# GANtastic3/MaskCycleGAN-VC

Measured on AMD Instinct MI355X. Metric: train iters/s (full G+D step), 80x64 mel bs=1, higher is better.
Workload: dtype f32

## Files before the change

### maskcyclegan-vc_amd/csrc/trunk.h

```cpp
#pragma once
#include <hip/hip_runtime.h>

enum TrunkMode { TRUNK_PLAIN = 0, TRUNK_IN = 1, TRUNK_IN_GLU = 2 };

struct TrunkArgs {
    const float* a0; const float* a1;
    const float* bias0; const float* bias1;
    const float* x; long long x_sc; long long x_sb;
    int Cin, KW, K;
    int M, Mtot;
    int B, T4, N;
    float* conv_out; long long c_sc; long long c_sb;
    int accumulate;
    int slab_all;
    float* slabs; long long slab_stride;
    float* stats;
    const float* gamma0; const float* beta0; const float* gamma1; const float* beta1;
    float* y; const float* res; long long y_sn; long long y_sc;
    float eps;
    int mode;
    int pre;
    int pre_C;
    const float* pre_x;
    int pre_xB;
// ... 17 lines not shown
    float* stats;
    float* y; long long y_sn, y_sc;
    const float* res;
    int Cin, KW, M, mode;
    int rows;
};
#define MCVC_TRUNK_NET_LAYERS 13
struct TrunkFwdNetArgs {
    TrunkLayerDesc L[MCVC_TRUNK_NET_LAYERS];
    int nlayers, B, T4;
    int x_floats;
    float eps;
    unsigned* sync;
    int fault_inject;
};
int mcvc_trunk_set_fault_inject(int on);
int mcvc_trunk_set_passes_in_flight(int n);
bool mcvc_trunk_net_applies(int B, int T4);
int mcvc_trunk_fwd_net_launch(TrunkFwdNetArgs& a, hipStream_t s);
#define MCVC_TRUNK_SYNC_WORDS 32

struct TrunkBwdLayerDesc {
    const float* wt;
    const float* dy;
    const float* px;
    int pxB;
    const float* stats;
    const float* g0; const float* b0; const float* g1; const float* b1;
    float* xout;
    float* dg0; float* db0; float* dg1; float* db1;
    float* out;
    int pre, C, M, rows;
    int flags;
};
enum { TBWD_ACCUMULATE = 1,
       TBWD_DY_FRESH = 2,
       TBWD_SLAB_DY = 4, TBWD_SLAB_OUT = 8 };
#define MCVC_TRUNK_BWD_LAYERS 12
struct TrunkBwdNetArgs {
    TrunkBwdLayerDesc L[MCVC_TRUNK_BWD_LAYERS];
    int nlayers, B, T4, x_floats;
    const float* slabs; long long slab_stride; int nslab;
    unsigned* sync;
    unsigned* err;
    int fault_inject;
};
bool mcvc_trunk_bwd_net_applies(int B, int T4);
int mcvc_trunk_bwd_net_launch(TrunkBwdNetArgs& a, hipStream_t s);
```

### maskcyclegan-vc_amd/csrc/trunk_kernels.hip

```cpp
#include "mcvc_common.h"
#include "trace.h"
#include "launch.h"
#include "trunk.h"

#define MFMA16(a, b, c) __builtin_amdgcn_mfma_f32_16x16x4f32((a), (b), (c), 0, 0, 0)

namespace {

constexpr int kTrunkWaves = 8;
constexpr int kTrunkThreads = 64 * kTrunkWaves;

__host__ __device__ inline int trunk_doff(int KW) { return KW == 3 ? 4 : 0; }
__host__ __device__ inline int trunk_tp(int T4, int KW) { return T4 + trunk_doff(KW); }
__host__ __device__ inline int trunk_rs(int B, int T4, int KW)
{
    int rs = B * trunk_tp(T4, KW);
    if (KW == 3) { while ((rs & 7) != 4) ++rs; }
    else { while ((rs & 3) != 2) ++rs; }
    return rs;
}
__host__ __device__ inline int trunk_na(int N) { return (N + 15) >> 4; }
constexpr int kRedPitch = 80;
__host__ __device__ inline int trunk_epi_floats(int NA) { return kTrunkWaves * NA * 4 * kRedPitch + 16 * (16 * NA + 1) + 16 * 8 * 2 + 16; }

// ... 600 lines not shown
                if (!ok) __hip_atomic_store(a.sync + MCVC_TRUNK_SYNC_WORDS - 1, 1u + (unsigned)l, __ATOMIC_RELAXED, __HIP_MEMORY_SCOPE_AGENT);
                flag[0] = ok ? 1.f : 0.f;
            }
            asm volatile("s_waitcnt lgkmcnt(0)" ::: "memory");
            __builtin_amdgcn_s_barrier();
            if (flag[0] == 0.f) {
                const TrunkLayerDesc& dl = a.L[a.nlayers - 1];
                const int N = a.B * a.T4;
                for (int tile = blockIdx.x; tile < dl.M / dl.rows; tile += gridDim.x)
                    for (int i = tid; i < dl.rows * N; i += kNetThreads) {
                        const int row = i / N, col = i - row * N, b = col / a.T4, t = col - b * a.T4;
                        dl.y[(long long)b * dl.y_sn + (long long)(tile * dl.rows + row) * dl.y_sc + t] = __builtin_nanf("");
                    }
                return;
            }
        }
        if (d.KW == 3) net_stage_x<3>(d.x, Xs, d.Cin, a.B, a.T4, tid, l > 0); else net_stage_x<1>(d.x, Xs, d.Cin, a.B, a.T4, tid, l > 0);
        __syncthreads();
        const bool wt = (l + 1 < a.nlayers);
        for (int tile = blockIdx.x; tile < ntiles; tile += gridDim.x) {
            if (tile != (int)blockIdx.x) { if (d.KW == 3) net_load_w<3>(d, tile, w3); else net_load_w<1>(d, tile, w1); net_load_e(d, a.B, a.T4, tile, pe); }
            if (d.KW == 3) net_tile<3, NA>(d, a.B, a.T4, a.eps, tile, Xs, epi, wt, w3, pe);
            else net_tile<1, NA>(d, a.B, a.T4, a.eps, tile, Xs, epi, wt, w1, pe);
        }
        if (wt) {
            asm volatile("s_waitcnt vmcnt(0)" ::: "memory");
            __syncthreads();
            if (tid == 0 && !(a.fault_inject && l == 0 && blockIdx.x == 0))
                __hip_atomic_fetch_add(a.sync + l, 1u, __ATOMIC_RELAXED, __HIP_MEMORY_SCOPE_AGENT);
        }
    }
}

__device__ __forceinline__ void bnet_stage_pre(const TrunkBwdNetArgs& a, const TrunkBwdLayerDesc& d, float* Xs, float* rsum, int B, int T4, int tid)
{
    constexpr int DOFF = 4;
    const int TP = T4 + DOFF, RS = trunk_rs(B, T4, 3);
    const int C = d.C;
    const bool pglu = (d.pre == 2);
    const int Cx = pglu ? 2 * C : C;
    const int PB = d.pxB > 0 ? d.pxB : B;
    const float invT = 1.0f / (float)T4;
    const int E = (T4 + 3) >> 2;
    const int items = Cx * B * 4;
    const int nwg = (int)gridDim.x, me = (int)blockIdx.x;
    if (T4 == 16 && !(d.flags & TBWD_SLAB_DY) && ((reinterpret_cast<unsigned long long>(d.dy) | reinterpret_cast<unsigned long long>(d.px) |
                                                   reinterpret_cast<unsigned long long>(d.xout)) & 15ull) == 0) {
        constexpr int U = 4;
        const bool fresh = (d.flags & TBWD_DY_FRESH) != 0;
        const __amdgpu_buffer_rsrc_t rs = __builtin_amdgcn_make_buffer_rsrc(const_cast<float*>(d.dy), 0, C * B * 16 * 4, 0x00020000);
        for (int it0 = 0; it0 < items; it0 += U * kNetThreads) {
            float4 vd[U], v0[U], v1[U];
            float g0[U], b0[U], g1[U], b1[U], m0[U], r0[U], m1[U], r1[U];
#pragma unroll
            for (int u = 0; u < U; ++u) {
                const int item = it0 + u * kNetThreads + tid;
                const bool live = item < items;
                const int q4 = item & 3, row = live ? (item >> 2) : 0;
                const int cx = row / B, b = row - cx * B;
                const bool gate = pglu && cx >= C;
                const int c = gate ? cx - C : cx;
                const long long ro = ((long long)c * B + b) * 16 + q4 * 4;
                const long long po = ((long long)c * PB + b) * 16 + q4 * 4;
                vd[u] = fresh ? __builtin_bit_cast(float4, __builtin_amdgcn_raw_buffer_load_b128(rs, (int)(ro * 4), 0, 16))
                              : *reinterpret_cast<const float4*>(d.dy + ro);
                v0[u] = *reinterpret_cast<const float4*>(d.px + po);
                v1[u] = pglu ? *reinterpret_cast<const float4*>(d.px + po + (long long)C * PB * 16) : make_float4(0.f, 0.f, 0.f, 0.f);
                g0[u] = d.g0[c]; b0[u] = d.b0[c];
                g1[u] = pglu ? d.g1[c] : 0.f; b1[u] = pglu ? d.b1[c] : 0.f;
                const float* st = d.stats + (long long)b * Cx * 2;
                m0[u] = st[2 * c]; r0[u] = st[2 * c + 1];
                m1[u] = pglu ? st[2 * (c + C)] : 0.f; r1[u] = pglu ? st[2 * (c + C) + 1] : 1.f;
            }
#pragma unroll
            for (int u = 0; u < U; ++u) {
                const int item = it0 + u * kNetThreads + tid;
                const bool live = item < items;
                const int q4 = item & 3, row = live ? (item >> 2) : 0;
                const int cx = row / B, b = row - cx * B;
                const bool gate = pglu && cx >= C;
                const float dv[4] = {vd[u].x, vd[u].y, vd[u].z, vd[u].w};
                const float x0[4] = {v0[u].x, v0[u].y, v0[u].z, v0[u].w};
                const float x1[4] = {v1[u].x, v1[u].y, v1[u].z, v1[u].w};
                float dzv[4], xhv[4];
                float s1 = 0.f, s2 = 0.f;
#pragma unroll
                for (int e = 0; e < 4; ++e) {
                    const float xh0 = (x0[e] - m0[u]) * r0[u];
                    float dz, xh;
                    if (pglu) {
                        const float xh1 = (x1[e] - m1[u]) * r1[u];
                        const float sg = sigmoidf_(xh1 * g1[u] + b1[u]);
                        if (gate) { dz = dv[e] * (xh0 * g0[u] + b0[u]) * sg * (1.0f - sg); xh = xh1; }
                        else { dz = dv[e] * sg; xh = xh0; }
                    } else { dz = dv[e]; xh = xh0; }
                    dzv[e] = live ? dz : 0.f; xhv[e] = live ? xh : 0.f;
                    s1 += dzv[e]; s2 += dzv[e] * xhv[e];
                }
                s1 += __shfl_xor(s1, 1, 64); s2 += __shfl_xor(s2, 1, 64);
                s1 += __shfl_xor(s1, 2, 64); s2 += __shfl_xor(s2, 2, 64);
                if (live) {
                    const bool mine = (cx % nwg) == me;
                    const float gr = gate ? g1[u] * r1[u] : g0[u] * r0[u];
                    float o[4];
#pragma unroll
                    for (int e = 0; e < 4; ++e) o[e] = gr * (dzv[e] - s1 * invT - xhv[e] * (s2 * invT));
                    *reinterpret_cast<float4*>(Xs + cx * RS + b * TP + DOFF + q4 * 4) = make_float4(o[0], o[1], o[2], o[3]);
                    if (mine) *reinterpret_cast<float4*>(d.xout + ((long long)cx * B + b) * 16 + q4 * 4) = make_float4(o[0], o[1], o[2], o[3]);
                    if (q4 == 0 && mine) { rsum[((cx / nwg) * B + b) * 2] = s1; rsum[((cx / nwg) * B + b) * 2 + 1] = s2; }
                }
            }
        }
    } else
    for (int it0 = 0; it0 < items; it0 += kNetThreads) {
        const int item = it0 + tid;
        const bool live = item < items;
        const int q4 = item & 3, row = live ? (item >> 2) : 0;
        const int cx = row / B, b = row - cx * B;
        const bool gate = pglu && cx >= C;
        const int c = gate ? cx - C : cx;
        const float g0 = d.g0[c], b0 = d.b0[c];
        const float g1 = pglu ? d.g1[c] : 0.f, b1 = pglu ? d.b1[c] : 0.f;
        const float* st = d.stats + (long long)b * Cx * 2;
        const float m0 = st[2 * c], r0 = st[2 * c + 1];
        const float m1 = pglu ? st[2 * (c + C)] : 0.f, r1 = pglu ? st[2 * (c + C) + 1] : 1.f;
        const int t0 = q4 * E;
        const float* dyr = d.dy + ((long long)c * B + b) * T4 + t0;
        const float* x0r = d.px + ((long long)c * PB + b) * T4 + t0;
        const float* x1r = d.px + ((long long)(c + C) * PB + b) * T4 + t0;
        float vd[8], v0[8], v1[8];
#pragma unroll
        for (int e = 0; e < 8; ++e) {
            const bool ok = live && e < E && (t0 + e) < T4;
            vd[e] = ok ? ((d.flags & TBWD_DY_FRESH) ? __hip_atomic_load(dyr + e, __ATOMIC_RELAXED, __HIP_MEMORY_SCOPE_AGENT) : dyr[e]) : 0.f;
            if (ok && (d.flags & TBWD_SLAB_DY))
                for (int sl = 1; sl < a.nslab; ++sl) vd[e] += a.slabs[(long long)(sl - 1) * a.slab_stride + ((long long)c * B + b) * T4 + t0 + e];
            v0[e] = ok ? x0r[e] : 0.f; v1[e] = (ok && pglu) ? x1r[e] : 0.f;
        }
        float dzv[8], xhv[8];
        float s1 = 0.f, s2 = 0.f;
#pragma unroll
        for (int e = 0; e < 8; ++e) {
            const bool ok = e < E && (t0 + e) < T4;
            const float xh0 = (v0[e] - m0) * r0;
            float dz, xh;
            if (pglu) {
                const float xh1 = (v1[e] - m1) * r1;
                const float sg = sigmoidf_(xh1 * g1 + b1);
                if (gate) { dz = vd[e] * (xh0 * g0 + b0) * sg * (1.0f - sg); xh = xh1; }
                else { dz = vd[e] * sg; xh = xh0; }
            } else { dz = vd[e]; xh = xh0; }
            dzv[e] = ok ? dz : 0.f; xhv[e] = ok ? xh : 0.f;
            s1 += dzv[e]; s2 += dzv[e] * xhv[e];
        }
        s1 += __shfl_xor(s1, 1, 64); s2 += __shfl_xor(s2, 1, 64);
        s1 += __shfl_xor(s1, 2, 64); s2 += __shfl_xor(s2, 2, 64);
        if (live) {
            const bool mine = (cx % nwg) == me;
            const float gr = gate ? g1 * r1 : g0 * r0;
            float* xrow = Xs + cx * RS + b * TP + DOFF;
            float* od = mine ? (d.xout + ((long long)cx * B + b) * T4 + t0) : nullptr;
#pragma unroll
            for (int e = 0; e < 8; ++e) {
                if (e < E && (t0 + e) < T4) {
                    const float dxv = gr * (dzv[e] - s1 * invT - xhv[e] * (s2 * invT));
                    xrow[t0 + e] = dxv;
                    if (od) od[e] = dxv;
                }
            }
            if (q4 == 0 && mine) { rsum[((cx / nwg) * B + b) * 2] = s1; rsum[((cx / nwg) * B + b) * 2 + 1] = s2; }
        }
    }
    trunk_zero_gaps(Xs, Cx, B, TP, RS, DOFF, tid, kNetThreads);
    __syncthreads();
    for (int j = tid; j * nwg + me < Cx; j += kNetThreads) {
        const int cx = j * nwg + me;
        const bool gate = pglu && cx >= C;
        const int c = gate ? cx - C : cx;
        float dgam = 0.f, dbet = 0.f;
        for (int b = 0; b < B; ++b) { dbet += rsum[(j * B + b) * 2]; dgam += rsum[(j * B + b) * 2 + 1]; }
        float* dg = gate ? d.dg1 : d.dg0;
        float* db = gate ? d.db1 : d.db0;
        if (dg) dg[c] += dgam;
        if (db) db[c] += dbet;
    }
}

template <int NA>
__device__ __forceinline__ void bnet_tile(const TrunkBwdLayerDesc& d, int B, int T4, int tile, const float* Xs, float* epi, bool wt,
                                          NetW<3>& pre, float old)
{
    constexpr int KW = 3, DOFF = 4;
    const int tid = threadIdx.x;
    const int lane = tid & 63;
    const int wave = __builtin_amdgcn_readfirstlane(tid >> 6);
    const int l15 = lane & 15, kq = lane >> 4;
    const int TP = T4 + DOFF, RS = trunk_rs(B, T4, 3);
    const int N = B * T4;
    const int Cx = (d.pre == 2) ? 2 * d.C : d.C;
    const int K = Cx * KW;
    const int rows = d.rows, r0 = tile * rows;
    const int k_count = K / kNetWaves;
    const int k_begin = wave * k_count;
    const float* arow = d.wt + (long long)(r0 + (l15 < rows ? l15 : rows - 1)) * K;
    constexpr int NQ = 3, GK = 48, CH = 4;
    const int sgroups = k_count / GK;
    const float* ap = arow + k_begin + 4 * NQ * kq;
    float4 (&wb)[CH][3] = pre.wb;
    int off[NA][NQ][4];
#pragma unroll
    for (int h = 0; h < NA; ++h) {
        const int n = l15 + 16 * h;
        int xcol = B * TP, live = 0;
        if (n < N) { const int b = n / T4, t = n - b * T4; xcol = b * TP + DOFF - 1 + t; live = 1; }
#pragma unroll
        for (int q = 0; q < NQ; ++q)
#pragma unroll
            for (int j = 0; j < 4; ++j) {
                const int kr = 4 * (NQ * kq + q) + j;
                off[h][q][j] = (kr / KW) * RS + xcol + (live ? (kr % KW) : 0);
            }
    }
    f32x4 acc[NA];
#pragma unroll
    for (int h = 0; h < NA; ++h) acc[h] = f32x4{0.f, 0.f, 0.f, 0.f};
    {
        const float* xs = Xs + (k_begin / KW) * RS;
        for (int sg0 = 0; sg0 < sgroups; sg0 += CH) {
            if (sg0 > 0) {
#pragma unroll
                for (int c = 0; c < CH; ++c) {
                    const float* pp = ap + (long long)(sg0 + c < sgroups ? sg0 + c : 0) * GK;
#pragma unroll
                    for (int q = 0; q < NQ; ++q) wb[c][q] = *reinterpret_cast<const float4*>(pp + 4 * q);
                }
            }
#pragma unroll
            for (int c = 0; c < CH; ++c) {
                if (sg0 + c < sgroups) {
                    float xv[NQ][4][NA];
#pragma unroll
                    for (int q = 0; q < NQ; ++q)
#pragma unroll
                        for (int j = 0; j < 4; ++j)
#pragma unroll
                            for (int h = 0; h < NA; ++h) xv[q][j][h] = xs[off[h][q][j]];
#pragma unroll
                    for (int q = 0; q < NQ; ++q) {
                        const float av[4] = {wb[c][q].x, wb[c][q].y, wb[c][q].z, wb[c][q].w};
#pragma unroll
                        for (int j = 0; j < 4; ++j)
#pragma unroll
                            for (int h = 0; h < NA; ++h) acc[h] = MFMA16(av[j], xv[q][j][h], acc[h]);
                    }
                    __builtin_amdgcn_sched_group_barrier(0x100, NQ * 4 * NA, 0);
                    __builtin_amdgcn_sched_group_barrier(0x008, NQ * 4 * NA, 0);
                    xs += (GK / KW) * RS;
                }
            }
        }
    }
    float* red = epi;
#pragma unroll
    for (int h = 0; h < NA; ++h)
#pragma unroll
        for (int r = 0; r < 4; ++r) red[((wave * NA + h) * 4 + r) * kRedPitch + lane] = acc[h][r];
    __syncthreads();
    if (tid < rows * N) {
        const int mrow = tid / N, col = tid - mrow * N;
        const int h = col >> 4, ln = ((mrow >> 2) << 4) + (col & 15), r = mrow & 3;
        float v = 0.f;
#pragma unroll
        for (int w = 0; w < kNetWaves; ++w) v += red[((w * NA + h) * 4 + r) * kRedPitch + ln];
        if (d.flags & TBWD_ACCUMULATE) v += old;
        float* dst = d.out + (long long)(r0 + mrow) * N + col;
        if (wt) st_wt(dst, v); else *dst = v;
    }
}

static_assert(sizeof(Twin<TrunkBwdNetArgs>) <= 4096 && sizeof(Twin<TrunkFwdNetArgs>) <= 4096, "kernel arguments are limited to 4 KB");
template <int NA>
__global__ void __launch_bounds__(kNetThreads) trunk_bwd_net_kernel(const Twin<TrunkBwdNetArgs> tw)
{
    const TrunkBwdNetArgs& a = tw.v[blockIdx.z];
    extern __shared__ __attribute__((aligned(16))) float smem[];
    float* Xs = smem;
    float* rsum = smem + a.x_floats;
    float* epi = rsum + 16 * 8 * 2 * 2;
    float* flag = epi + kNetWaves * NA * 4 * kRedPitch;
    const int tid = threadIdx.x;
    const int N = a.B * a.T4;
    for (int l = 0; l < a.nlayers; ++l) {
        const TrunkBwdLayerDesc d = a.L[l];
        const int ntiles = d.M / d.rows;
        const int Cx = (d.pre == 2) ? 2 * d.C : d.C;
        NetW<3> w3;
        TrunkLayerDesc wd{};
        wd.a0 = d.wt; wd.Cin = Cx; wd.KW = 3; wd.M = d.M; wd.mode = TRUNK_PLAIN; wd.rows = d.rows;
        const bool mine = (int)blockIdx.x < ntiles;
        float old = 0.f;
        auto load_old = [&](int tile) {
            float v = 0.f;
            if ((d.flags & TBWD_ACCUMULATE) && tid < d.rows * N) {
                const long long idx = (long long)(tile * d.rows) * N + tid;
                v = __hip_atomic_load(d.out + idx, __ATOMIC_RELAXED, __HIP_MEMORY_SCOPE_AGENT);
                if (d.flags & TBWD_SLAB_OUT)
                    for (int sl = 1; sl < a.nslab; ++sl) v += a.slabs[(long long)(sl - 1) * a.slab_stride + idx];
            }
            return v;
        };
        if (mine) {
            net_load_w<3>(wd, blockIdx.x, w3);
            old = load_old(blockIdx.x);
        }
        if (l > 0) {
            if (tid == 0) {
                const bool ok = wait_arrivals(a.sync + (l - 1), gridDim.x);
                if (!ok) __hip_atomic_store(a.err, 0x100u + (unsigned)l, __ATOMIC_RELAXED, __HIP_MEMORY_SCOPE_AGENT);
                flag[0] = ok ? 1.f : 0.f;
            }
            asm volatile("s_waitcnt lgkmcnt(0)" ::: "memory");
            __builtin_amdgcn_s_barrier();
            if (flag[0] == 0.f) {
                const TrunkBwdLayerDesc& dl = a.L[a.nlayers - 1];
                for (int tile = blockIdx.x; tile < dl.M / dl.rows; tile += gridDim.x)
                    for (int i = tid; i < dl.rows * N; i += kNetThreads) dl.out[(long long)(tile * dl.rows) * N + i] = __builtin_nanf("");
                return;
            }
        }
        bnet_stage_pre(a, d, Xs, rsum, a.B, a.T4, tid);
        __syncthreads();
        const bool wt = (l + 1 < a.nlayers);
        for (int tile = blockIdx.x; tile < ntiles; tile += gridDim.x) {
            if (tile != (int)blockIdx.x) {
                net_load_w<3>(wd, tile, w3);
                old = load_old(tile);
            }
            bnet_tile<NA>(d, a.B, a.T4, tile, Xs, epi, wt, w3, old);
        }
        if (wt) {
            asm volatile("s_waitcnt vmcnt(0)" ::: "memory");
            __syncthreads();
            if (tid == 0 && !(a.fault_inject && l == 0 && blockIdx.x == 0))
                __hip_atomic_fetch_add(a.sync + l, 1u, __ATOMIC_RELAXED, __HIP_MEMORY_SCOPE_AGENT);
        }
    }
}

struct ZeroWordsKArgs { unsigned* p; int n; };
__global__ void zero_words_kernel(const Twin<ZeroWordsKArgs> tw)
{
    const ZeroWordsKArgs a = tw.v[blockIdx.z];
    if ((int)threadIdx.x < a.n) a.p[threadIdx.x] = 0u;
}

struct FillRowsKArgs { float* dst; const float* bias; int C; int per_row; };
__global__ void __launch_bounds__(256) fill_rows_kernel(const Twin<FillRowsKArgs> tw)
{
    const FillRowsKArgs ka_ = tw.v[blockIdx.z];
    float* __restrict__ dst = ka_.dst;
    const float* __restrict__ bias = ka_.bias;
    int C = ka_.C;
    int per_row = ka_.per_row;
    const int i = blockIdx.x * 256 + threadIdx.x;
    if (i >= C * per_row) return;
    dst[i] = bias ? bias[i / per_row] : 0.f;
}

}

int mcvc_fill_rows_launch(float* dst, const float* bias, int C, int per_row, hipStream_t s)
{
    TraceScope ts(K_ELEMENTWISE, s, 0.0, 4.0 * C * per_row);
    mcvc_launch(fill_rows_kernel, dim3((unsigned)cdiv_i(C * per_row, 256)), dim3(256), 0, s, FillRowsKArgs{dst, bias, C, per_row});
    return (int)hipGetLastError();
}

// ... 39 lines not shown
}

template <int KW>
static int trunk_launch_k(const TrunkArgs& a, dim3 grid, size_t lds, hipStream_t s)
{
    switch (trunk_na(a.N)) {
    case 1: return trunk_launch_t<KW, 1>(a, grid, lds, s);
    case 2: return trunk_launch_t<KW, 2>(a, grid, lds, s);
    case 3: return trunk_launch_t<KW, 3>(a, grid, lds, s);
    default: return trunk_launch_t<KW, 4>(a, grid, lds, s);
    }
}

int mcvc_trunk_launch(const TrunkArgs& a, int ksplit, hipStream_t s)
{
    if (!mcvc_trunk_applies(a.Cin, a.KW, a.M, a.B, a.T4, a.mode, ksplit)) return MCVC_ERR_INVALID;
    if (ksplit > 1 && !(a.mode == TRUNK_PLAIN && (a.accumulate || a.slabs))) return MCVC_ERR_INVALID;
    if (a.slab_all && !(a.mode == TRUNK_PLAIN && a.slabs)) return MCVC_ERR_INVALID;
    if (a.pre && (a.mode != TRUNK_PLAIN || a.T4 > 32 || !a.pre_x || !a.pre_stats || !a.pre_out || (a.pre_xB > 0 && a.pre_xB < a.B))) return MCVC_ERR_INVALID;
    const int rows = (a.mode == TRUNK_IN_GLU) ? 8 : 16;
    dim3 grid((unsigned)(a.M / rows), (unsigned)ksplit);
    size_t lds = (size_t)mcvc_trunk_lds_floats(a.Cin, a.KW, a.B, a.T4, ksplit) * sizeof(float);
    if (a.pre) {
        const long long xs = (long long)(a.Cin / ksplit) * trunk_rs(a.B, a.T4, a.KW) + 4 + (long long)(a.Cin / ksplit) * a.B * 2;
        if ((size_t)xs * sizeof(float) > lds) lds = (size_t)xs * sizeof(float);
        if (lds > 160 * 1024) return MCVC_ERR_INVALID;
    }
    const double mt = (a.mode == TRUNK_IN_GLU) ? 2.0 * a.M : (double)a.M;
    TraceScope ts(K_TRUNK, s, 2.0 * mt * a.K * a.N, 4.0 * (mt * a.K + (double)a.Cin * a.N + 3.0 * mt * a.N));
    return a.KW == 3 ? trunk_launch_k<3>(a, grid, lds, s) : trunk_launch_k<1>(a, grid, lds, s);
}

static long long net_fwd_lds_floats(int B, int T4) { return (long long)512 * trunk_rs(B, T4, 3) + 4 + trunk_epi_floats(trunk_na(B * T4)); }
static long long net_bwd_lds_floats(int B, int T4) { return (long long)1024 * trunk_rs(B, T4, 3) + 4 + 16 * 8 * 2 * 2 + kNetWaves * trunk_na(B * T4) * 4 * kRedPitch + 16; }

static int g_trunk_passes_in_flight = 2;
static int device_cus()
{
    static const int n = [] { int dev = 0, v = 0; if (hipGetDevice(&dev) != hipSuccess || hipDeviceGetAttribute(&v, hipDeviceAttributeMultiprocessorCount, dev) != hipSuccess) v = 0; return v; }();
    return n;
}
int mcvc_trunk_set_passes_in_flight(int n) { const int was = g_trunk_passes_in_flight; if (n >= 1) g_trunk_passes_in_flight = n; return was; }
static bool trunk_residency_ok() { const int cus = device_cus(); return cus <= 0 || kNetGrid * g_trunk_passes_in_flight <= cus; }

bool mcvc_trunk_net_applies(int B, int T4)
{
    if (B < 1 || B > 8 || T4 < 1 || T4 > 32 || B * T4 > 48) return false;
    return trunk_residency_ok() && net_fwd_lds_floats(B, T4) * 4 <= 160 * 1024;
}

bool mcvc_trunk_bwd_net_applies(int B, int T4)
{
    if (B < 1 || B > 8 || T4 < 4 || T4 > 32 || B * T4 > 32) return false;
    return trunk_residency_ok() && net_bwd_lds_floats(B, T4) * 4 <= 160 * 1024;
}

static int g_trunk_fault_inject = 0;
int mcvc_trunk_set_fault_inject(int on) { const int was = g_trunk_fault_inject; g_trunk_fault_inject = on ? 1 : 0; return was; }

int mcvc_trunk_fwd_net_launch(TrunkFwdNetArgs& a, hipStream_t s)
{
    if (!mcvc_trunk_net_applies(a.B, a.T4) || a.nlayers < 1 || a.nlayers > MCVC_TRUNK_NET_LAYERS || !a.sync) return MCVC_ERR_INVALID;
    long long xmax = 0;
    double flops = 0.0, bytes = 0.0;
    const int N = a.B * a.T4;
    for (int l = 0; l < a.nlayers; ++l) {
        const TrunkLayerDesc& d = a.L[l];
        if (d.KW != 1 && d.KW != 3) return MCVC_ERR_INVALID;
        const int K = d.Cin * d.KW, gk = (d.KW == 3) ? 48 : 32;
        if (K % (gk * kNetWaves) != 0 || d.rows < 1 || d.rows > 16 || d.M % d.rows != 0) return MCVC_ERR_INVALID;
        if (d.mode == TRUNK_IN_GLU && d.rows > 8) return MCVC_ERR_INVALID;
        if (d.mode != TRUNK_IN_GLU && d.mode != TRUNK_IN) return MCVC_ERR_INVALID;
        const int rows_tot = d.mode == TRUNK_IN_GLU ? 2 * d.rows : d.rows;
        if (d.rows * N > kNetThreads || rows_tot * N > 2 * kNetThreads) return MCVC_ERR_INVALID;
        const long long x = (long long)d.Cin * trunk_rs(a.B, a.T4, d.KW) + 4;
        if (x > xmax) xmax = x;
        const double mt = (d.mode == TRUNK_IN_GLU) ? 2.0 * d.M : (double)d.M;
        flops += 2.0 * mt * K * N;
        bytes += 4.0 * (mt * K + (double)d.Cin * N + 3.0 * mt * N);
    }
    a.x_floats = (int)((xmax + 3) & ~3LL);
    a.fault_inject = g_trunk_fault_inject;
    const int NA = trunk_na(N);
    const size_t lds = ((size_t)a.x_floats + trunk_epi_floats(NA)) * sizeof(float);
    if (lds > 160 * 1024) return MCVC_ERR_INVALID;
    hipError_t e = hipSuccess;
    mcvc_launch(zero_words_kernel, dim3(1), dim3(64), 0, s, ZeroWordsKArgs{a.sync, MCVC_TRUNK_SYNC_WORDS - 1});
    TraceScope ts(K_TRUNK, s, flops, bytes);
    static bool done[4] = {false, false, false, false};
    typedef void (*KernT)(const Twin<TrunkFwdNetArgs>);
    const KernT fns[4] = {nullptr, trunk_fwd_net_kernel<1>, trunk_fwd_net_kernel<2>, trunk_fwd_net_kernel<3>};
    if (!done[NA]) {
        e = hipFuncSetAttribute(reinterpret_cast<const void*>(fns[NA]), hipFuncAttributeMaxDynamicSharedMemorySize, 160 * 1024);
        if (e != hipSuccess) return (int)e;
        done[NA] = true;
    }
    mcvc_launch(fns[NA], dim3(kNetGrid), dim3(kNetThreads), lds, s, a);
    return (int)hipGetLastError();
}

int mcvc_trunk_bwd_net_launch(TrunkBwdNetArgs& a, hipStream_t s)
{
    if (!mcvc_trunk_bwd_net_applies(a.B, a.T4) || a.nlayers < 1 || a.nlayers > MCVC_TRUNK_BWD_LAYERS || !a.sync || !a.err) return MCVC_ERR_INVALID;
    long long xmax = 0;
    double flops = 0.0, bytes = 0.0;
    const int N = a.B * a.T4;
    for (int l = 0; l < a.nlayers; ++l) {
        const TrunkBwdLayerDesc& d = a.L[l];
        const int Cx = (d.pre == 2) ? 2 * d.C : d.C;
        const int K = Cx * 3;
        if ((d.pre != 1 && d.pre != 2) || Cx > 1024 || K % (48 * kNetWaves) != 0 || d.rows < 1 || d.rows > 16 || d.M % d.rows != 0 || d.rows * N > kNetThreads ||
            (d.pxB > 0 && d.pxB < a.B))
            return MCVC_ERR_INVALID;
        const long long x = (long long)Cx * trunk_rs(a.B, a.T4, 3) + 4;
        if (x > xmax) xmax = x;
        flops += 2.0 * d.M * K * N;
        bytes += 4.0 * ((double)d.M * K + 3.0 * Cx * N + 2.0 * d.M * N);
    }
    a.x_floats = (int)((xmax + 3) & ~3LL);
    a.fault_inject = g_trunk_fault_inject;
    const bool wide = N > 16;
    const size_t lds = ((size_t)a.x_floats + 16 * 8 * 2 * 2 + kNetWaves * (wide ? 2 : 1) * 4 * kRedPitch + 16) * sizeof(float);
    if (lds > 160 * 1024) return MCVC_ERR_INVALID;
    mcvc_launch(zero_words_kernel, dim3(1), dim3(64), 0, s, ZeroWordsKArgs{a.sync, MCVC_TRUNK_SYNC_WORDS - 1});
    TraceScope ts(K_TRUNK, s, flops, bytes);
    static bool done[2] = {false, false};
    if (!done[wide]) {
        const void* fn = wide ? reinterpret_cast<const void*>(trunk_bwd_net_kernel<2>) : reinterpret_cast<const void*>(trunk_bwd_net_kernel<1>);
        hipError_t e = hipFuncSetAttribute(fn, hipFuncAttributeMaxDynamicSharedMemorySize, 160 * 1024);
        if (e != hipSuccess) return (int)e;
        done[wide] = true;
    }
    if (wide) mcvc_launch(trunk_bwd_net_kernel<2>, dim3(kNetGrid), dim3(kNetThreads), lds, s, a);
    else mcvc_launch(trunk_bwd_net_kernel<1>, dim3(kNetGrid), dim3(kNetThreads), lds, s, a);
    return (int)hipGetLastError();
}
```

Before: 176.4.

## Fuse next-layer IN/GLU backward prologue into trunk backward tile epilogue

Restructures the persistent trunk backward kernel. Each layer used to recompute the full pre-activation gradient (IN/GLU backward) for all channels in every workgroup. Now the owning tile's epilogue computes x' for the next layer's channels and writes it to global memory, and the next layer stages it from there. An initial pre-phase handles layer 0. Support is also added for chunking the K dimension when the staged activations do not fit in LDS. This removes redundant per-workgroup recomputation and global reads of dy/px/stats, at the cost of an extra global round-trip of x' and tighter layer-chaining constraints.

```diff
diff --git a/maskcyclegan-vc_amd/csrc/trunk.h b/maskcyclegan-vc_amd/csrc/trunk.h
--- a/maskcyclegan-vc_amd/csrc/trunk.h
+++ b/maskcyclegan-vc_amd/csrc/trunk.h
@@ -73,6 +73,7 @@
     float* out;
     int pre, C, M, rows;
     int flags;
+    int nchunk;
 };
 enum { TBWD_ACCUMULATE = 1,
        TBWD_DY_FRESH = 2,
diff --git a/maskcyclegan-vc_amd/csrc/trunk_kernels.hip b/maskcyclegan-vc_amd/csrc/trunk_kernels.hip
--- a/maskcyclegan-vc_amd/csrc/trunk_kernels.hip
+++ b/maskcyclegan-vc_amd/csrc/trunk_kernels.hip
@@ -656,151 +656,75 @@
     }
 }
 
-__device__ __forceinline__ void bnet_stage_pre(const TrunkBwdNetArgs& a, const TrunkBwdLayerDesc& d, float* Xs, float* rsum, int B, int T4, int tid)
-{
-    constexpr int DOFF = 4;
-    const int TP = T4 + DOFF, RS = trunk_rs(B, T4, 3);
-    const int C = d.C;
+
+struct BnetXP { float g0, b0, g1, b1, m0, r0, m1, r1; float x0[8], x1[8]; };
+
+__device__ __forceinline__ void bnet_load_xp(const TrunkBwdLayerDesc& d, int B, int T4, int c, int b, int q4, bool live, BnetXP& p)
+{
     const bool pglu = (d.pre == 2);
-    const int Cx = pglu ? 2 * C : C;
+    const int C = d.C, Cx = pglu ? 2 * C : C;
     const int PB = d.pxB > 0 ? d.pxB : B;
+    p.g0 = d.g0[c]; p.b0 = d.b0[c];
+    p.g1 = pglu ? d.g1[c] : 0.f; p.b1 = pglu ? d.b1[c] : 0.f;
+    const float* st = d.stats + (long long)b * Cx * 2;
+    p.m0 = st[2 * c]; p.r0 = st[2 * c + 1];
+    p.m1 = pglu ? st[2 * (c + C)] : 0.f; p.r1 = pglu ? st[2 * (c + C) + 1] : 1.f;
+    const int E = (T4 + 3) >> 2, t0 = q4 * E;
+    const float* x0r = d.px + ((long long)c * PB + b) * T4 + t0;
+    const float* x1r = d.px + ((long long)(c + C) * PB + b) * T4 + t0;
+#pragma unroll
+    for (int e = 0; e < 8; ++e) {
+        const bool ok = live && e < E && (t0 + e) < T4;
+        p.x0[e] = ok ? x0r[e] : 0.f; p.x1[e] = (ok && pglu) ? x1r[e] : 0.f;
+    }
+}
+
+__device__ __forceinline__ void bnet_xprime(const float (&vd)[8], const BnetXP& p, bool pglu, bool gate, int T4, int q4, float (&o)[8], float& s1, float& s2)
+{
     const float invT = 1.0f / (float)T4;
-    const int E = (T4 + 3) >> 2;
-    const int items = Cx * B * 4;
-    const int nwg = (int)gridDim.x, me = (int)blockIdx.x;
-    if (T4 == 16 && !(d.flags & TBWD_SLAB_DY) && ((reinterpret_cast<unsigned long long>(d.dy) | reinterpret_cast<unsigned long long>(d.px) |
-                                                   reinterpret_cast<unsigned long long>(d.xout)) & 15ull) == 0) {
-        constexpr int U = 4;
-        const bool fresh = (d.flags & TBWD_DY_FRESH) != 0;
-        const __amdgpu_buffer_rsrc_t rs = __builtin_amdgcn_make_buffer_rsrc(const_cast<float*>(d.dy), 0, C * B * 16 * 4, 0x00020000);
-        for (int it0 = 0; it0 < items; it0 += U * kNetThreads) {
-            float4 vd[U], v0[U], v1[U];
-            float g0[U], b0[U], g1[U], b1[U], m0[U], r0[U], m1[U], r1[U];
-#pragma unroll
-            for (int u = 0; u < U; ++u) {
-                const int item = it0 + u * kNetThreads + tid;
-                const bool live = item < items;
-                const int q4 = item & 3, row = live ? (item >> 2) : 0;
-                const int cx = row / B, b = row - cx * B;
-                const bool gate = pglu && cx >= C;
-                const int c = gate ? cx - C : cx;
-                const long long ro = ((long long)c * B + b) * 16 + q4 * 4;
-                const long long po = ((long long)c * PB + b) * 16 + q4 * 4;
-                vd[u] = fresh ? __builtin_bit_cast(float4, __builtin_amdgcn_raw_buffer_load_b128(rs, (int)(ro * 4), 0, 16))
-                              : *reinterpret_cast<const float4*>(d.dy + ro);
-                v0[u] = *reinterpret_cast<const float4*>(d.px + po);
-                v1[u] = pglu ? *reinterpret_cast<const float4*>(d.px + po + (long long)C * PB * 16) : make_float4(0.f, 0.f, 0.f, 0.f);
-                g0[u] = d.g0[c]; b0[u] = d.b0[c];
-                g1[u] = pglu ? d.g1[c] : 0.f; b1[u] = pglu ? d.b1[c] : 0.f;
-                const float* st = d.stats + (long long)b * Cx * 2;
-                m0[u] = st[2 * c]; r0[u] = st[2 * c + 1];
-                m1[u] = pglu ? st[2 * (c + C)] : 0.f; r1[u] = pglu ? st[2 * (c + C) + 1] : 1.f;
-            }
-#pragma unroll
-            for (int u = 0; u < U; ++u) {
-                const int item = it0 + u * kNetThreads + tid;
-                const bool live = item < items;
-                const int q4 = item & 3, row = live ? (item >> 2) : 0;
-                const int cx = row / B, b = row - cx * B;
-                const bool gate = pglu && cx >= C;
-                const float dv[4] = {vd[u].x, vd[u].y, vd[u].z, vd[u].w};
-                const float x0[4] = {v0[u].x, v0[u].y, v0[u].z, v0[u].w};
-                const float x1[4] = {v1[u].x, v1[u].y, v1[u].z, v1[u].w};
-                float dzv[4], xhv[4];
-                float s1 = 0.f, s2 = 0.f;
-#pragma unroll
-                for (int e = 0; e < 4; ++e) {
-                    const float xh0 = (x0[e] - m0[u]) * r0[u];
-                    float dz, xh;
-                    if (pglu) {
-                        const float xh1 = (x1[e] - m1[u]) * r1[u];
-                        const float sg = sigmoidf_(xh1 * g1[u] + b1[u]);
-                        if (gate) { dz = dv[e] * (xh0 * g0[u] + b0[u]) * sg * (1.0f - sg); xh = xh1; }
-                        else { dz = dv[e] * sg; xh = xh0; }
-                    } else { dz = dv[e]; xh = xh0; }
-                    dzv[e] = live ? dz : 0.f; xhv[e] = live ? xh : 0.f;
-                    s1 += dzv[e]; s2 += dzv[e] * xhv[e];
-                }
-                s1 += __shfl_xor(s1, 1, 64); s2 += __shfl_xor(s2, 1, 64);
-                s1 += __shfl_xor(s1, 2, 64); s2 += __shfl_xor(s2, 2, 64);
-                if (live) {
-                    const bool mine = (cx % nwg) == me;
-                    const float gr = gate ? g1[u] * r1[u] : g0[u] * r0[u];
-                    float o[4];
-#pragma unroll
-                    for (int e = 0; e < 4; ++e) o[e] = gr * (dzv[e] - s1 * invT - xhv[e] * (s2 * invT));
-                    *reinterpret_cast<float4*>(Xs + cx * RS + b * TP + DOFF + q4 * 4) = make_float4(o[0], o[1], o[2], o[3]);
-                    if (mine) *reinterpret_cast<float4*>(d.xout + ((long long)cx * B + b) * 16 + q4 * 4) = make_float4(o[0], o[1], o[2], o[3]);
-                    if (q4 == 0 && mine) { rsum[((cx / nwg) * B + b) * 2] = s1; rsum[((cx / nwg) * B + b) * 2 + 1] = s2; }
-                }
-            }
-        }
-    } else
-    for (int it0 = 0; it0 < items; it0 += kNetThreads) {
-        const int item = it0 + tid;
-        const bool live = item < items;
-        const int q4 = item & 3, row = live ? (item >> 2) : 0;
-        const int cx = row / B, b = row - cx * B;
-        const bool gate = pglu && cx >= C;
-        const int c = gate ? cx - C : cx;
-        const float g0 = d.g0[c], b0 = d.b0[c];
-        const float g1 = pglu ? d.g1[c] : 0.f, b1 = pglu ? d.b1[c] : 0.f;
-        const float* st = d.stats + (long long)b * Cx * 2;
-        const float m0 = st[2 * c], r0 = st[2 * c + 1];
-        const float m1 = pglu ? st[2 * (c + C)] : 0.f, r1 = pglu ? st[2 * (c + C) + 1] : 1.f;
-        const int t0 = q4 * E;
-        const float* dyr = d.dy + ((long long)c * B + b) * T4 + t0;
-        const float* x0r = d.px + ((long long)c * PB + b) * T4 + t0;
-        const float* x1r = d.px + ((long long)(c + C) * PB + b) * T4 + t0;
-        float vd[8], v0[8], v1[8];
-#pragma unroll
-        for (int e = 0; e < 8; ++e) {
-            const bool ok = live && e < E && (t0 + e) < T4;
-            vd[e] = ok ? ((d.flags & TBWD_DY_FRESH) ? __hip_atomic_load(dyr + e, __ATOMIC_RELAXED, __HIP_MEMORY_SCOPE_AGENT) : dyr[e]) : 0.f;
-            if (ok && (d.flags & TBWD_SLAB_DY))
-                for (int sl = 1; sl < a.nslab; ++sl) vd[e] += a.slabs[(long long)(sl - 1) * a.slab_stride + ((long long)c * B + b) * T4 + t0 + e];
-            v0[e] = ok ? x0r[e] : 0.f; v1[e] = (ok && pglu) ? x1r[e] : 0.f;
-        }
-        float dzv[8], xhv[8];
-        float s1 = 0.f, s2 = 0.f;
-#pragma unroll
-        for (int e = 0; e < 8; ++e) {
-            const bool ok = e < E && (t0 + e) < T4;
-            const float xh0 = (v0[e] - m0) * r0;
-            float dz, xh;
-            if (pglu) {
-                const float xh1 = (v1[e] - m1) * r1;
-                const float sg = sigmoidf_(xh1 * g1 + b1);
-                if (gate) { dz = vd[e] * (xh0 * g0 + b0) * sg * (1.0f - sg); xh = xh1; }
-                else { dz = vd[e] * sg; xh = xh0; }
-            } else { dz = vd[e]; xh = xh0; }
-            dzv[e] = ok ? dz : 0.f; xhv[e] = ok ? xh : 0.f;
-            s1 += dzv[e]; s2 += dzv[e] * xhv[e];
-        }
-        s1 += __shfl_xor(s1, 1, 64); s2 += __shfl_xor(s2, 1, 64);
-        s1 += __shfl_xor(s1, 2, 64); s2 += __shfl_xor(s2, 2, 64);
-        if (live) {
-            const bool mine = (cx % nwg) == me;
-            const float gr = gate ? g1 * r1 : g0 * r0;
-            float* xrow = Xs + cx * RS + b * TP + DOFF;
-            float* od = mine ? (d.xout + ((long long)cx * B + b) * T4 + t0) : nullptr;
-#pragma unroll
-            for (int e = 0; e < 8; ++e) {
-                if (e < E && (t0 + e) < T4) {
-                    const float dxv = gr * (dzv[e] - s1 * invT - xhv[e] * (s2 * invT));
-                    xrow[t0 + e] = dxv;
-                    if (od) od[e] = dxv;
-                }
-            }
-            if (q4 == 0 && mine) { rsum[((cx / nwg) * B + b) * 2] = s1; rsum[((cx / nwg) * B + b) * 2 + 1] = s2; }
-        }
-    }
-    trunk_zero_gaps(Xs, Cx, B, TP, RS, DOFF, tid, kNetThreads);
-    __syncthreads();
-    for (int j = tid; j * nwg + me < Cx; j += kNetThreads) {
-        const int cx = j * nwg + me;
-        const bool gate = pglu && cx >= C;
-        const int c = gate ? cx - C : cx;
+    const int E = (T4 + 3) >> 2, t0 = q4 * E;
+    float dzv[8], xhv[8];
+    s1 = 0.f; s2 = 0.f;
+#pragma unroll
+    for (int e = 0; e < 8; ++e) {
+        const bool ok = e < E && (t0 + e) < T4;
+        const float xh0 = (p.x0[e] - p.m0) * p.r0;
+        float dz, xh;
+        if (pglu) {
+            const float xh1 = (p.x1[e] - p.m1) * p.r1;
+            const float sg = sigmoidf_(xh1 * p.g1 + p.b1);
+            if (gate) { dz = vd[e] * (xh0 * p.g0 + p.b0) * sg * (1.0f - sg); xh = xh1; }
+            else { dz = vd[e] * sg; xh = xh0; }
+        } else { dz = vd[e]; xh = xh0; }
+        dzv[e] = ok ? dz : 0.f; xhv[e] = ok ? xh : 0.f;
+        s1 += dzv[e]; s2 += dzv[e] * xhv[e];
+    }
+    s1 += __shfl_xor(s1, 1, 64); s2 += __shfl_xor(s2, 1, 64);
+    s1 += __shfl_xor(s1, 2, 64); s2 += __shfl_xor(s2, 2, 64);
+    const float gr = gate ? p.g1 * p.r1 : p.g0 * p.r0;
+#pragma unroll
+    for (int e = 0; e < 8; ++e) o[e] = gr * (dzv[e] - s1 * invT - xhv[e] * (s2 * invT));
+}
+
+__device__ __forceinline__ void bnet_store_xprime(const TrunkBwdLayerDesc& d, int B, int T4, int cx, int b, int q4, const float (&o)[8], float s1, float s2,
+                                                  float* rs)
+{
+    const int E = (T4 + 3) >> 2, t0 = q4 * E;
+    float* od = d.xout + ((long long)cx * B + b) * T4 + t0;
+#pragma unroll
+    for (int e = 0; e < 8; ++e)
+        if (e < E && (t0 + e) < T4) st_wt(od + e, o[e]);
+    if (q4 == 0) { rs[0] = s1; rs[1] = s2; }
+}
+
+template <typename F>
+__device__ __forceinline__ void bnet_affine_grads(const TrunkBwdLayerDesc& d, int B, const float* rsum, int n, F chan)
+{
+    const bool pglu = (d.pre == 2);
+    for (int j = threadIdx.x; j < n; j += kNetThreads) {
+        const int cx = chan(j);
+        const bool gate = pglu && cx >= d.C;
+        const int c = gate ? cx - d.C : cx;
         float dgam = 0.f, dbet = 0.f;
         for (int b = 0; b < B; ++b) { dbet += rsum[(j * B + b) * 2]; dgam += rsum[(j * B + b) * 2 + 1]; }
         float* dg = gate ? d.dg1 : d.dg0;
@@ -810,25 +734,115 @@
     }
 }
 
+__device__ __forceinline__ void bnet_pre_phase(const TrunkBwdNetArgs& a, const TrunkBwdLayerDesc& d, float* rsum, int B, int T4)
+{
+    const int tid = threadIdx.x;
+    const bool pglu = (d.pre == 2);
+    const int C = d.C, Cx = pglu ? 2 * C : C;
+    const int nwg = (int)gridDim.x, me = (int)blockIdx.x;
+    const int nown = me < Cx ? (Cx - me + nwg - 1) / nwg : 0;
+    const int items = nown * B * 4;
+    const int E = (T4 + 3) >> 2;
+    for (int it0 = 0; it0 < items; it0 += kNetThreads) {
+        const int item = it0 + tid;
+        const bool live = item < items;
+        const int q4 = item & 3, row = live ? (item >> 2) : 0;
+        const int j = row / B, b = row - j * B;
+        const int cx = live ? j * nwg + me : 0;
+        const bool gate = pglu && cx >= C;
+        const int c = gate ? cx - C : cx;
+        BnetXP p;
+        bnet_load_xp(d, B, T4, c, b, q4, live, p);
+        const int t0 = q4 * E;
+        const float* dyr = d.dy + ((long long)c * B + b) * T4 + t0;
+        float vd[8];
+#pragma unroll
+        for (int e = 0; e < 8; ++e) {
+            const bool ok = live && e < E && (t0 + e) < T4;
+            vd[e] = ok ? dyr[e] : 0.f;
+            if (ok && (d.flags & TBWD_SLAB_DY))
+                for (int sl = 1; sl < a.nslab; ++sl) vd[e] += a.slabs[(long long)(sl - 1) * a.slab_stride + ((long long)c * B + b) * T4 + t0 + e];
+        }
+        float o[8], s1, s2;
+        bnet_xprime(vd, p, pglu, gate, T4, q4, o, s1, s2);
+        if (live) bnet_store_xprime(d, B, T4, cx, b, q4, o, s1, s2, rsum + (j * B + b) * 2);
+    }
+    __syncthreads();
+    bnet_affine_grads(d, B, rsum, nown, [&](int j) { return j * nwg + me; });
+}
+
+struct BnetItem { int xi, b, q4, c, cx; bool gate, live; };
+__device__ __forceinline__ BnetItem bnet_item(const TrunkBwdLayerDesc& dn, int r0, int rows, int B)
+{
+    const int tid = threadIdx.x;
+    const bool pglu = (dn.pre == 2);
+    const int nxc = pglu ? 2 * rows : rows;
+    BnetItem it;
+    it.live = tid < nxc * B * 4;
+    it.q4 = tid & 3;
+    const int row = it.live ? (tid >> 2) : 0;
+    it.xi = row / B; it.b = row - it.xi * B;
+    it.gate = pglu && it.xi >= rows;
+    it.c = r0 + (it.gate ? it.xi - rows : it.xi);
+    it.cx = it.gate ? dn.C + it.c : it.c;
+    return it;
+}
+
+__device__ __forceinline__ void bnet_stage(const float* __restrict__ xsrc, float* Xs, int Cx, int nc, int ch, int B, int T4, int tid)
+{
+    constexpr int DOFF = 4;
+    const int TP = T4 + DOFF, RS = trunk_rs(B, T4, 3);
+    const int nch = Cx / nc, P = nch / kNetWaves, W = Cx / kNetWaves;
+    auto src_row = [&](int j) { return nc == 1 ? j : (j / P) * W + ch * P + (j - (j / P) * P); };
+    if (((T4 & 3) == 0) && ((reinterpret_cast<unsigned long long>(xsrc) & 15ull) == 0)) {
+        const int nf4 = (nch * B * T4) >> 2;
+        const __amdgpu_buffer_rsrc_t rsrc = __builtin_amdgcn_make_buffer_rsrc(const_cast<float*>(xsrc), 0, Cx * B * T4 * 4, 0x00020000);
+        for (int f0 = 0; f0 < nf4; f0 += 4 * kNetThreads) {
+            float4 v[4];
+#pragma unroll
+            for (int u = 0; u < 4; ++u) {
+                const int f = f0 + u * kNetThreads + tid;
+                const int e = 4 * f, r = e / T4, t = e - r * T4;
+                const int j = r / B, b = r - j * B;
+                const int so = f < nf4 ? ((src_row(j) * B + b) * T4 + t) * 4 : Cx * B * T4 * 4;
+                v[u] = __builtin_bit_cast(float4, __builtin_amdgcn_raw_buffer_load_b128(rsrc, so, 0, 16));
+            }
+#pragma unroll
+            for (int u = 0; u < 4; ++u) {
+                const int f = f0 + u * kNetThreads + tid;
+                if (f < nf4) {
+                    const int e = 4 * f, r = e / T4, t = e - r * T4;
+                    const int j = r / B, b = r - j * B;
+                    *reinterpret_cast<float4*>(Xs + j * RS + b * TP + DOFF + t) = v[u];
+                }
+            }
+        }
+    } else {
+        for (int i = tid; i < nch * B * T4; i += kNetThreads) {
+            const int r = i / T4, t = i - r * T4;
+            const int j = r / B, b = r - j * B;
+            Xs[j * RS + b * TP + DOFF + t] = __hip_atomic_load(xsrc + ((long long)src_row(j) * B + b) * T4 + t, __ATOMIC_RELAXED, __HIP_MEMORY_SCOPE_AGENT);
+        }
+    }
+    trunk_zero_gaps(Xs, nch, B, TP, RS, DOFF, tid, kNetThreads);
+}
+
 template <int NA>
-__device__ __forceinline__ void bnet_tile(const TrunkBwdLayerDesc& d, int B, int T4, int tile, const float* Xs, float* epi, bool wt,
-                                          NetW<3>& pre, float old)
+__device__ __forceinline__ void bnet_kpart(const TrunkBwdLayerDesc& d, int B, int T4, int tile, const float* Xs, int P, int s0, int s1, NetW<3>& pre,
+                                           f32x4 (&acc)[NA])
 {
     constexpr int KW = 3, DOFF = 4;
-    const int tid = threadIdx.x;
-    const int lane = tid & 63;
-    const int wave = __builtin_amdgcn_readfirstlane(tid >> 6);
+    const int lane = threadIdx.x & 63;
+    const int wave = __builtin_amdgcn_readfirstlane((int)threadIdx.x >> 6);
     const int l15 = lane & 15, kq = lane >> 4;
     const int TP = T4 + DOFF, RS = trunk_rs(B, T4, 3);
     const int N = B * T4;
     const int Cx = (d.pre == 2) ? 2 * d.C : d.C;
     const int K = Cx * KW;
     const int rows = d.rows, r0 = tile * rows;
-    const int k_count = K / kNetWaves;
-    const int k_begin = wave * k_count;
+    const int k_begin = wave * (K / kNetWaves);
     const float* arow = d.wt + (long long)(r0 + (l15 < rows ? l15 : rows - 1)) * K;
     constexpr int NQ = 3, GK = 48, CH = 4;
-    const int sgroups = k_count / GK;
     const float* ap = arow + k_begin + 4 * NQ * kq;
     float4 (&wb)[CH][3] = pre.wb;
     int off[NA][NQ][4];
@@ -845,45 +859,51 @@
                 off[h][q][j] = (kr / KW) * RS + xcol + (live ? (kr % KW) : 0);
             }
     }
-    f32x4 acc[NA];
-#pragma unroll
-    for (int h = 0; h < NA; ++h) acc[h] = f32x4{0.f, 0.f, 0.f, 0.f};
-    {
-        const float* xs = Xs + (k_begin / KW) * RS;
-        for (int sg0 = 0; sg0 < sgroups; sg0 += CH) {
-            if (sg0 > 0) {
-#pragma unroll
-                for (int c = 0; c < CH; ++c) {
-                    const float* pp = ap + (long long)(sg0 + c < sgroups ? sg0 + c : 0) * GK;
-#pragma unroll
-                    for (int q = 0; q < NQ; ++q) wb[c][q] = *reinterpret_cast<const float4*>(pp + 4 * q);
+    const float* xs = Xs + wave * P * RS;
+    for (int sg0 = s0; sg0 < s1; sg0 += CH) {
+        if (sg0 > 0) {
+#pragma unroll
+            for (int c = 0; c < CH; ++c) {
+                const float* pp = ap + (long long)(sg0 + c < s1 ? sg0 + c : s0) * GK;
+#pragma unroll
+                for (int q = 0; q < NQ; ++q) wb[c][q] = *reinterpret_cast<const float4*>(pp + 4 * q);
+            }
+        }
+#pragma unroll
+        for (int c = 0; c < CH; ++c) {
+            if (sg0 + c < s1) {
+                float xv[NQ][4][NA];
+#pragma unroll
+                for (int q = 0; q < NQ; ++q)
+#pragma unroll
+                    for (int j = 0; j < 4; ++j)
+#pragma unroll
+                        for (int h = 0; h < NA; ++h) xv[q][j][h] = xs[off[h][q][j]];
+#pragma unroll
+                for (int q = 0; q < NQ; ++q) {
+                    const float av[4] = {wb[c][q].x, wb[c][q].y, wb[c][q].z, wb[c][q].w};
+#pragma unroll
+                    for (int j = 0; j < 4; ++j)
+#pragma unroll
+                        for (int h = 0; h < NA; ++h) acc[h] = MFMA16(av[j], xv[q][j][h], acc[h]);
                 }
-            }
-#pragma unroll
-            for (int c = 0; c < CH; ++c) {
-                if (sg0 + c < sgroups) {
-                    float xv[NQ][4][NA];
-#pragma unroll
-                    for (int q = 0; q < NQ; ++q)
-#pragma unroll
-                        for (int j = 0; j < 4; ++j)
-#pragma unroll
-                            for (int h = 0; h < NA; ++h) xv[q][j][h] = xs[off[h][q][j]];
-#pragma unroll
-                    for (int q = 0; q < NQ; ++q) {
-                        const float av[4] = {wb[c][q].x, wb[c][q].y, wb[c][q].z, wb[c][q].w};
-#pragma unroll
-                        for (int j = 0; j < 4; ++j)
-#pragma unroll
-                            for (int h = 0; h < NA; ++h) acc[h] = MFMA16(av[j], xv[q][j][h], acc[h]);
-                    }
-                    __builtin_amdgcn_sched_group_barrier(0x100, NQ * 4 * NA, 0);
-                    __builtin_amdgcn_sched_group_barrier(0x008, NQ * 4 * NA, 0);
-                    xs += (GK / KW) * RS;
-                }
-            }
-        }
-    }
+                __builtin_amdgcn_sched_group_barrier(0x100, NQ * 4 * NA, 0);
+                __builtin_amdgcn_sched_group_barrier(0x008, NQ * 4 * NA, 0);
+                xs += (GK / KW) * RS;
+            }
+        }
+    }
+}
+
+template <int NA>
+__device__ __forceinline__ void bnet_epilogue(const TrunkBwdLayerDesc& d, const TrunkBwdLayerDesc& dn, bool next, int B, int T4, int tile, float* epi, float* ytile,
+                                              float* rsum, bool wt, float old, const f32x4 (&acc)[NA], const BnetXP& xp)
+{
+    const int tid = threadIdx.x;
+    const int lane = tid & 63;
+    const int wave = __builtin_amdgcn_readfirstlane(tid >> 6);
+    const int N = B * T4;
+    const int rows = d.rows, r0 = tile * rows;
     float* red = epi;
 #pragma unroll
     for (int h = 0; h < NA; ++h)
@@ -899,7 +919,24 @@
         if (d.flags & TBWD_ACCUMULATE) v += old;
         float* dst = d.out + (long long)(r0 + mrow) * N + col;
         if (wt) st_wt(dst, v); else *dst = v;
-    }
+        if (next) ytile[tid] = v;
+    }
+    if (!next) return;
+    __syncthreads();
+    const BnetItem it = bnet_item(dn, r0, rows, B);
+    const bool pglu = (dn.pre == 2);
+    const int E = (T4 + 3) >> 2, t0 = it.q4 * E;
+    float vd[8];
+#pragma unroll
+    for (int e = 0; e < 8; ++e) {
+        const bool ok = it.live && e < E && (t0 + e) < T4;
+        vd[e] = ok ? ytile[(it.c - r0) * N + it.b * T4 + t0 + e] : 0.f;
+    }
+    float o[8], s1, s2;
+    bnet_xprime(vd, xp, pglu, it.gate, T4, it.q4, o, s1, s2);
+    if (it.live) bnet_store_xprime(dn, B, T4, it.cx, it.b, it.q4, o, s1, s2, rsum + (it.xi * B + it.b) * 2);
+    __syncthreads();
+    bnet_affine_grads(dn, B, rsum, pglu ? 2 * rows : rows, [&](int xi) { return xi < rows ? r0 + xi : dn.C + r0 + xi - rows; });
 }
 
 static_assert(sizeof(Twin<TrunkBwdNetArgs>) <= 4096 && sizeof(Twin<TrunkFwdNetArgs>) <= 4096, "kernel arguments are limited to 4 KB");
@@ -910,15 +947,25 @@
     extern __shared__ __attribute__((aligned(16))) float smem[];
     float* Xs = smem;
     float* rsum = smem + a.x_floats;
-    float* epi = rsum + 16 * 8 * 2 * 2;
+    float* ytile = rsum + 512;
+    float* epi = ytile + 512;
     float* flag = epi + kNetWaves * NA * 4 * kRedPitch;
     const int tid = threadIdx.x;
     const int N = a.B * a.T4;
+    bnet_pre_phase(a, a.L[0], rsum, a.B, a.T4);
+    asm volatile("s_waitcnt vmcnt(0)" ::: "memory");
+    __syncthreads();
+    if (tid == 0 && !(a.fault_inject && blockIdx.x == 0))
+        __hip_atomic_fetch_add(a.sync, 1u, __ATOMIC_RELAXED, __HIP_MEMORY_SCOPE_AGENT);
     for (int l = 0; l < a.nlayers; ++l) {
         const TrunkBwdLayerDesc d = a.L[l];
+        const bool next = (l + 1 < a.nlayers);
+        const TrunkBwdLayerDesc& dn = a.L[next ? l + 1 : l];
         const int ntiles = d.M / d.rows;
         const int Cx = (d.pre == 2) ? 2 * d.C : d.C;
+        const int nc = d.nchunk, sgroups = Cx * 3 / kNetWaves / 48, P = Cx / kNetWaves / nc;
         NetW<3> w3;
+        BnetXP xp;
         TrunkLayerDesc wd{};
         wd.a0 = d.wt; wd.Cin = Cx; wd.KW = 3; wd.M = d.M; wd.mode = TRUNK_PLAIN; wd.rows = d.rows;
         const bool mine = (int)blockIdx.x < ntiles;
@@ -933,40 +980,58 @@
             }
             return v;
         };
+        auto load_xp = [&](int tile) {
+            if (!next) return;
+            const BnetItem it = bnet_item(dn, tile * d.rows, d.rows, a.B);
+            bnet_load_xp(dn, a.B, a.T4, it.c, it.b, it.q4, it.live, xp);
+        };
         if (mine) {
             net_load_w<3>(wd, blockIdx.x, w3);
             old = load_old(blockIdx.x);
-        }
-        if (l > 0) {
-            if (tid == 0) {
-                const bool ok = wait_arrivals(a.sync + (l - 1), gridDim.x);
-                if (!ok) __hip_atomic_store(a.err, 0x100u + (unsigned)l, __ATOMIC_RELAXED, __HIP_MEMORY_SCOPE_AGENT);
-                flag[0] = ok ? 1.f : 0.f;
-            }
-            asm volatile("s_waitcnt lgkmcnt(0)" ::: "memory");
-            __builtin_amdgcn_s_barrier();
-            if (flag[0] == 0.f) {
-                const TrunkBwdLayerDesc& dl = a.L[a.nlayers - 1];
-                for (int tile = blockIdx.x; tile < dl.M / dl.rows; tile += gridDim.x)
-                    for (int i = tid; i < dl.rows * N; i += kNetThreads) dl.out[(long long)(tile * dl.rows) * N + i] = __builtin_nanf("");
-                return;
-            }
-        }
-        bnet_stage_pre(a, d, Xs, rsum, a.B, a.T4, tid);
-        __syncthreads();
-        const bool wt = (l + 1 < a.nlayers);
+            load_xp(blockIdx.x);
+        }
+        if (tid == 0) {
+            const bool ok = wait_arrivals(a.sync + l, gridDim.x);
+            if (!ok) __hip_atomic_store(a.err, 0x100u + (unsigned)l, __ATOMIC_RELAXED, __HIP_MEMORY_SCOPE_AGENT);
+            flag[0] = ok ? 1.f : 0.f;
+        }
+        asm volatile("s_waitcnt lgkmcnt(0)" ::: "memory");
+        __builtin_amdgcn_s_barrier();
+        if (flag[0] == 0.f) {
+            const TrunkBwdLayerDesc& dl = a.L[a.nlayers - 1];
+            for (int tile = blockIdx.x; tile < dl.M / dl.rows; tile += gridDim.x)
+                for (int i = tid; i < dl.rows * N; i += kNetThreads) dl.out[(long long)(tile * dl.rows) * N + i] = __builtin_nanf("");
+            return;
+        }
+        if (nc == 1) {
+            bnet_stage(d.xout, Xs, Cx, 1, 0, a.B, a.T4, tid);
+            __syncthreads();
+        }
+        const bool wt = next;
         for (int tile = blockIdx.x; tile < ntiles; tile += gridDim.x) {
             if (tile != (int)blockIdx.x) {
                 net_load_w<3>(wd, tile, w3);
                 old = load_old(tile);
-            }
-            bnet_tile<NA>(d, a.B, a.T4, tile, Xs, epi, wt, w3, old);
+                load_xp(tile);
+            }
+            f32x4 acc[NA];
+#pragma unroll
+            for (int h = 0; h < NA; ++h) acc[h] = f32x4{0.f, 0.f, 0.f, 0.f};
+            for (int ch = 0; ch < nc; ++ch) {
+                if (nc > 1) {
+                    __syncthreads();
+                    bnet_stage(d.xout, Xs, Cx, nc, ch, a.B, a.T4, tid);
+                    __syncthreads();
+                }
+                bnet_kpart<NA>(d, a.B, a.T4, tile, Xs, P, ch * (sgroups / nc), (ch + 1) * (sgroups / nc), w3, acc);
+            }
+            bnet_epilogue<NA>(d, dn, next, a.B, a.T4, tile, epi, ytile, rsum, wt, old, acc, xp);
+            __syncthreads();
         }
         if (wt) {
             asm volatile("s_waitcnt vmcnt(0)" ::: "memory");
             __syncthreads();
-            if (tid == 0 && !(a.fault_inject && l == 0 && blockIdx.x == 0))
-                __hip_atomic_fetch_add(a.sync + l, 1u, __ATOMIC_RELAXED, __HIP_MEMORY_SCOPE_AGENT);
+            if (tid == 0) __hip_atomic_fetch_add(a.sync + l + 1, 1u, __ATOMIC_RELAXED, __HIP_MEMORY_SCOPE_AGENT);
         }
     }
 }
@@ -1072,7 +1137,15 @@
 }
 
 static long long net_fwd_lds_floats(int B, int T4) { return (long long)512 * trunk_rs(B, T4, 3) + 4 + trunk_epi_floats(trunk_na(B * T4)); }
-static long long net_bwd_lds_floats(int B, int T4) { return (long long)1024 * trunk_rs(B, T4, 3) + 4 + 16 * 8 * 2 * 2 + kNetWaves * trunk_na(B * T4) * 4 * kRedPitch + 16; }
+static long long net_bwd_fixed_floats(int N) { return 512 + 512 + kNetWaves * trunk_na(N) * 4 * kRedPitch + 16; }
+static long long net_bwd_x_floats(int Cx, int nc, int B, int T4) { return ((long long)(Cx / nc) * trunk_rs(B, T4, 3) + 4 + 3) & ~3LL; }
+static int net_bwd_chunks(int Cx, int B, int T4)
+{
+    const int sg = Cx * 3 / (48 * kNetWaves);
+    for (int nc = 1; nc <= sg; nc *= 2)
+        if (sg % nc == 0 && (net_bwd_x_floats(Cx, nc, B, T4) + net_bwd_fixed_floats(B * T4)) * 4 <= 160 * 1024) return nc;
+    return 0;
+}
 
 static int g_trunk_passes_in_flight = 2;
 static int device_cus()
@@ -1092,7 +1165,7 @@
 bool mcvc_trunk_bwd_net_applies(int B, int T4)
 {
     if (B < 1 || B > 8 || T4 < 4 || T4 > 32 || B * T4 > 32) return false;
-    return trunk_residency_ok() && net_bwd_lds_floats(B, T4) * 4 <= 160 * 1024;
+    return trunk_residency_ok() && net_bwd_chunks(1024, B, T4) == 1 && net_bwd_chunks(256, B, T4) == 1;
 }
 
 static int g_trunk_fault_inject = 0;
@@ -1146,21 +1219,27 @@
     double flops = 0.0, bytes = 0.0;
     const int N = a.B * a.T4;
     for (int l = 0; l < a.nlayers; ++l) {
-        const TrunkBwdLayerDesc& d = a.L[l];
+        TrunkBwdLayerDesc& d = a.L[l];
         const int Cx = (d.pre == 2) ? 2 * d.C : d.C;
         const int K = Cx * 3;
         if ((d.pre != 1 && d.pre != 2) || Cx > 1024 || K % (48 * kNetWaves) != 0 || d.rows < 1 || d.rows > 16 || d.M % d.rows != 0 || d.rows * N > kNetThreads ||
             (d.pxB > 0 && d.pxB < a.B))
             return MCVC_ERR_INVALID;
-        const long long x = (long long)Cx * trunk_rs(a.B, a.T4, 3) + 4;
+        if (l > 0) {
+            const TrunkBwdLayerDesc& p = a.L[l - 1];
+            if (d.dy != p.out || d.C != p.M || (d.flags & TBWD_SLAB_DY) || (d.pre == 2 ? 2 : 1) * p.rows * a.B * 4 > kNetThreads) return MCVC_ERR_INVALID;
+        }
+        d.nchunk = net_bwd_chunks(Cx, a.B, a.T4);
+        if (d.nchunk < 1) return MCVC_ERR_INVALID;
+        const long long x = net_bwd_x_floats(Cx, d.nchunk, a.B, a.T4);
         if (x > xmax) xmax = x;
         flops += 2.0 * d.M * K * N;
         bytes += 4.0 * ((double)d.M * K + 3.0 * Cx * N + 2.0 * d.M * N);
     }
-    a.x_floats = (int)((xmax + 3) & ~3LL);
+    a.x_floats = (int)xmax;
     a.fault_inject = g_trunk_fault_inject;
     const bool wide = N > 16;
-    const size_t lds = ((size_t)a.x_floats + 16 * 8 * 2 * 2 + kNetWaves * (wide ? 2 : 1) * 4 * kRedPitch + 16) * sizeof(float);
+    const size_t lds = ((size_t)a.x_floats + net_bwd_fixed_floats(N)) * sizeof(float);
     if (lds > 160 * 1024) return MCVC_ERR_INVALID;
     mcvc_launch(zero_words_kernel, dim3(1), dim3(64), 0, s, ZeroWordsKArgs{a.sync, MCVC_TRUNK_SYNC_WORDS - 1});
     TraceScope ts(K_TRUNK, s, flops, bytes);
```

Result: no change. 177.5, median of 6 (+0.6%).
